# jaronlong52/neuron_poker

Measured on NVIDIA B200. Metric: showdown_evals_per_s, higher is better.
Workload: dtype u32

## Files before the change

### neuron_poker_b200/csrc/npk_device.cuh

```cuda
#pragma once
#include <cuda_runtime.h>
#include <stdint.h>

namespace npk {

constexpr int kDevDescShift = 9;
constexpr int kRowBits = 10;
constexpr uint32_t kColMask = (1u << kRowBits) - 1u;

struct DeviceTables {
    const uint16_t* value;
    const uint16_t* rowoff;
    const uint16_t* flush;
    const uint32_t* desc;
    uint32_t value_bytes;
    uint32_t rowoff_bytes;
    uint32_t flush_bytes;
    uint16_t type_start[10];
    uint32_t* check;
};

struct SmemTables {
    const uint16_t* value;
    const uint16_t* rowoff;
    const uint16_t* flush;
    const uint32_t* desc;
    uint32_t value_bytes, rowoff_bytes, flush_bytes;
    uint32_t* check;
};

#ifdef NPK_CHECKED
#define NPK_CHECK(ptr, cond, code) do { if (!(cond)) atomicMax((ptr), (unsigned)(code)); } while (0)
#else
#define NPK_CHECK(ptr, cond, code) do { } while (0)
#endif

constexpr uint32_t kDescBytes = 256;

__host__ __device__ __forceinline__ int validate_query(const uint8_t* hole, const uint8_t* board, int players,
                                                       unsigned long long* mask = nullptr)
{
    unsigned long long m = 0;
    int known = 0;
    bool bad = players < 1 || players > 10, ended = false;
    for (int i = 0; hole && i < 2; i++) {
        const int c = hole[i];
        if (c >= 52) bad = true; else { bad |= (m >> c & 1ull) != 0; m |= 1ull << c; }
    }
    for (int i = 0; i < 5; i++) {
        const int c = board[i];
        if (c == 0xFF) { ended = true; continue; }
        if (ended || c >= 52) { bad = true; continue; }
        bad |= (m >> c & 1ull) != 0;
        m |= 1ull << c;
        known++;
    }
    if (mask) *mask = m;
    return bad ? -1 : known;
}

__device__ __forceinline__ uint32_t smem_u32(const void* p) { return (uint32_t)__cvta_generic_to_shared(p); }

__device__ __forceinline__ void mbar_init(uint64_t* bar, uint32_t count)
{
    asm volatile("mbarrier.init.shared::cta.b64 [%0], %1;" ::"r"(smem_u32(bar)), "r"(count));
    asm volatile("fence.mbarrier_init.release.cluster;" ::: "memory");
}
__device__ __forceinline__ void mbar_expect_tx(uint64_t* bar, uint32_t bytes)
{
    asm volatile("mbarrier.arrive.expect_tx.shared::cta.b64 _, [%0], %1;" ::"r"(smem_u32(bar)), "r"(bytes) : "memory");
}
__device__ __forceinline__ void bulk_g2s(void* dst, const void* src, uint32_t bytes, uint64_t* bar)
{
    asm volatile("cp.async.bulk.shared::cluster.global.mbarrier::complete_tx::bytes [%0], [%1], %2, [%3];" ::"r"(
                     smem_u32(dst)),
                 "l"(src), "r"(bytes), "r"(smem_u32(bar))
                 : "memory");
}
__device__ __forceinline__ void mbar_wait(uint64_t* bar, uint32_t parity)
{
    uint32_t done = 0;
    while (!done) {
        asm volatile(
            "{\n .reg .pred p;\n mbarrier.try_wait.parity.shared::cta.b64 p, [%1], %2;\n selp.u32 %0, 1, 0, p;\n}\n"
            : "=r"(done)
            : "r"(smem_u32(bar)), "r"(parity)
            : "memory");
    }
}

__device__ __forceinline__ SmemTables stage_tables(const DeviceTables& t, uint8_t* base, uint64_t* bar)
{
    uint8_t* s_value = base;
    uint8_t* s_rowoff = s_value + t.value_bytes;
    uint8_t* s_flush = s_rowoff + t.rowoff_bytes;
    if (threadIdx.x == 0) mbar_init(bar, 1);
    __syncthreads();
    if (threadIdx.x == 0) {
        mbar_expect_tx(bar, t.value_bytes + t.rowoff_bytes + t.flush_bytes + kDescBytes);
        const uint32_t kChunk = 32768;
        for (uint32_t o = 0; o < t.value_bytes; o += kChunk)
            bulk_g2s(s_value + o, (const uint8_t*)t.value + o, min(kChunk, t.value_bytes - o), bar);
        bulk_g2s(s_rowoff, t.rowoff, t.rowoff_bytes, bar);
        bulk_g2s(s_flush, t.flush, t.flush_bytes, bar);
        bulk_g2s(s_flush + t.flush_bytes, t.desc, kDescBytes, bar);
    }
    mbar_wait(bar, 0);
    SmemTables s;
    s.value = (const uint16_t*)s_value;
    s.rowoff = (const uint16_t*)s_rowoff;
    s.flush = (const uint16_t*)s_flush;
    s.desc = (const uint32_t*)(s_flush + t.flush_bytes);
    s.value_bytes = t.value_bytes; s.rowoff_bytes = t.rowoff_bytes; s.flush_bytes = t.flush_bytes; s.check = t.check;
    return s;
}

__device__ __forceinline__ void philox4x32_10(uint32_t c0, uint32_t c1, uint32_t c2, uint32_t c3, uint32_t k0,
                                              uint32_t k1, uint32_t out[4])
{
    const uint32_t M0 = 0xD2511F53u, M1 = 0xCD9E8D57u, W0 = 0x9E3779B9u, W1 = 0xBB67AE85u;
#pragma unroll
    for (int r = 0; r < 10; r++) {
        uint64_t p0 = (uint64_t)M0 * c0, p1 = (uint64_t)M1 * c2;
        uint32_t n0 = (uint32_t)(p1 >> 32) ^ c1 ^ k0;
        uint32_t n2 = (uint32_t)(p0 >> 32) ^ c3 ^ k1;
        c1 = (uint32_t)p1;
        c3 = (uint32_t)p0;
        c0 = n0;
        c2 = n2;
        k0 += W0;
        k1 += W1;
    }
    out[0] = c0; out[1] = c1; out[2] = c2; out[3] = c3;
}

__device__ __forceinline__ uint32_t prmt(uint32_t a, uint32_t b, uint32_t sel)
{
    uint32_t r;
    asm("prmt.b32 %0, %1, %2, %3;" : "=r"(r) : "r"(a), "r"(b), "r"(sel));
    return r;
}

__device__ __forceinline__ uint32_t shr_clamp(uint32_t v, uint32_t n)
{
    uint32_t r;
    asm("shr.u32 %0, %1, %2;" : "=r"(r) : "r"(v), "r"(n));
    return r;
}

__device__ __forceinline__ uint32_t lds_u16(uint32_t saddr)
{
    uint32_t v;
    asm("ld.shared.u16 %0, [%1];" : "=r"(v) : "r"(saddr));
    return v;
}

struct SmemAddr {
    uint32_t value, rowoff, flush;
#ifdef NPK_CHECKED
    uint32_t value_bytes, rowoff_bytes, flush_bytes;
    uint32_t* check;
#endif
};

__device__ __forceinline__ SmemAddr smem_addr(const SmemTables& s)
{
    SmemAddr a;
    a.value = smem_u32(s.value); a.rowoff = smem_u32(s.rowoff); a.flush = smem_u32(s.flush);
#ifdef NPK_CHECKED
    a.value_bytes = s.value_bytes; a.rowoff_bytes = s.rowoff_bytes; a.flush_bytes = s.flush_bytes; a.check = s.check;
#endif
    return a;
}

__device__ __forceinline__ uint32_t lookup_nonflush(const SmemAddr& a, uint32_t total)
{
    const uint32_t row2 = __umulhi(total, 1u << (32 - (kDevDescShift + kRowBits - 1))) & (0xFFFFu << 1);
    NPK_CHECK(a.check, row2 + 2u <= a.rowoff_bytes, 1);
    const uint32_t off = lds_u16(a.rowoff + row2);
    const uint32_t col2 = __umulhi(total, 1u << (32 - (kDevDescShift - 1))) & (kColMask << 1);
    NPK_CHECK(a.check, col2 + (off << 1) + 2u <= a.value_bytes, 2);
    return lds_u16(a.value + col2 + (off << 1));
}

__device__ __forceinline__ uint32_t flush_bit(uint32_t d, uint32_t fsx) { return shr_clamp(0x1000u, (d ^ fsx) & 63u); }

__device__ __forceinline__ void card_bits(uint32_t d, uint32_t& lo, uint32_t& hi)
{
    const uint64_t b = 1ull << ((d & 0x30u) + 12u - (d & 15u));
    lo = (uint32_t)b;
    hi = (uint32_t)(b >> 32);
}

__device__ __forceinline__ uint32_t suit_inc(uint32_t d) { return 1u << ((d >> 2) & 12u); }

__device__ __forceinline__ uint32_t field_selector(uint32_t fs) { return 0x9910u + fs * 0x2222u; }

__device__ __forceinline__ uint32_t eval7_desc(const SmemAddr& a, const uint32_t d[7])
{
    uint32_t total = 0, cnt = 0x3333u;
#pragma unroll
    for (int i = 0; i < 7; i++) {
        total += d[i];
        cnt += suit_inc(d[i]);
    }
    uint32_t v = lookup_nonflush(a, total);
    const uint32_t f = cnt & 0x8888u;
    if (f) {
        const uint32_t fsx = (((31u - __clz(f)) >> 2) & 3u) << 4;
        uint32_t field = 0;
#pragma unroll
        for (int i = 0; i < 7; i++) field |= shr_clamp(0x1000u, (d[i] ^ fsx) & 63u);
        NPK_CHECK(a.check, 2u * field + 2u <= a.flush_bytes, 3);
        v = lds_u16(a.flush + 2u * field);
    }
    return v;
}

}
```

### neuron_poker_b200/csrc/npk_kernels.cu

```cuda
#include <atomic>
#include <cstdlib>
#include "npk_mc.cuh"

namespace npk {

template <int NOPP, int NB, int REF>
__device__ __forceinline__ void shape_kernel_body(const EquityParams& p)
{
    extern __shared__ __align__(128) uint8_t smem[];
    const WarpCtx cx = warp_context(p, smem, 64 + (45 + NB) * 32);
    const int lane = cx.lane;
    const long long n_items = p.nq * p.chunks;
    for (long long item = next_item(p.work_counter, lane); item < n_items; item = next_item(p.work_counter, lane)) {
        long long q, t_begin, t_end;
        item_range(p, item, q, t_begin, t_end);
        if (REF) refdeal_item<NOPP, NB>(p, cx, q, t_begin, t_end);
        else uniform_item<NOPP, NB>(p, cx, q, t_begin, t_end);
    }
    finish_single_call(p, lane);
    if (p.peer) finish_peer(p.peer, p.peer_epoch, p.peer_totals, p.peer_words, lane);
}

template <int NOPP, int NB>
__global__ void __launch_bounds__(kEquityMaxThreads, 1) equity_uniform_kernel(const EquityParams p)
{
    shape_kernel_body<NOPP, NB, 0>(p);
}

template <int NOPP, int NB>
__global__ void __launch_bounds__(kEquityMaxThreads, 1) equity_refdeal_kernel(const EquityParams p)
{
    shape_kernel_body<NOPP, NB, 1>(p);
}

__device__ __forceinline__ bool class_allowed(const uint32_t (&mask)[6], int c1, int c2)
{
    const int r1 = c1 >> 2, r2 = c2 >> 2, hi = max(r1, r2), lo = min(r1, r2);
    const int k = ((c1 ^ c2) & 3) == 0 ? hi * 13 + lo : lo * 13 + hi;
    return (mask[k >> 5] >> (k & 31)) & 1u;
}

template <int MODE>
__global__ void __launch_bounds__(kRefThreads, 1) equity_ranges_kernel(const EquityParams p)
{
    extern __shared__ __align__(128) uint8_t smem[];
    uint64_t* bar = reinterpret_cast<uint64_t*>(smem);
    const SmemAddr st = smem_addr(stage_tables(p.tables, smem + 128, bar));
    const int lane = threadIdx.x & 31;

    const long long n_items = p.nq * p.chunks;

    for (long long item = next_item(p.work_counter, lane); item < n_items; item = next_item(p.work_counter, lane)) {
        long long q, t_begin, t_end;
        item_range(p, item, q, t_begin, t_end);
        int known = 0;
        for (int i = 0; i < 5; i++) known += p.board[5 * q + i] != 0xFF;
        const int nknown = (int)p.n_known;
        const int nopp = max(0, (int)p.n_players[q] - 1 - nknown);

        uint64_t taken = 0;
        uint32_t board_sum = 0, board_lo = 0, board_hi = 0, board_cnt = 0x5555u;
        for (int i = 0; i < known; i++) {
            const uint8_t c = p.board[5 * q + i];
            const uint32_t d = p.tables.desc[c];
            uint32_t l, h;
            card_bits(d, l, h);
            board_sum += d; board_lo |= l; board_hi |= h; board_cnt += suit_inc(d);
            taken |= 1ull << c;
        }
        if (p.ghost)
            for (int i = 0; i < 2; i++) { const uint8_t c = p.ghost[2 * q + i]; if (c < 52) taken |= 1ull << c; }
        int h0 = 0, h1 = 0;
        if (!p.hero_range) { h0 = p.hole[2 * q]; h1 = p.hole[2 * q + 1]; taken |= (1ull << h0) | (1ull << h1); }
        for (int f = 0; f < 2 * nknown; f++) taken |= 1ull << (p.known_opp[2 * q * nknown + f] & 63u);
        const uint64_t avail0 = ~taken & ((1ull << 52) - 1ull);
        const int n0 = __popcll(avail0);

        uint32_t wins = 0, ties = 0;
        unsigned long long passes = 0;
        unsigned long long wt_pack = 0;

        for (long long tb = t_begin; tb < t_end; tb += 32) {
            if (*reinterpret_cast<volatile uint32_t*>(p.abort_flag)) break;
            const long long t_local = tb + lane;
            bool active = t_local < t_end;
            const unsigned long long trial = (unsigned long long)(p.trial_offset + t_local);
            WordStream rs;
            rs.c0 = (uint32_t)trial; rs.c1 = (uint32_t)(trial >> 32); rs.c2 = (uint32_t)q + p.query_offset;
            rs.k0 = p.seed_lo; rs.k1 = p.seed_hi; rs.blk = MODE == 1 ? 0x80000000u : 0xC0000000u; rs.have = 0;

            uint64_t avail = avail0;
            int n = n0;
            uint32_t hd0 = 0, hd1 = 0, best = 0;
            uint32_t oc1[9], oc2[9];
            if (active) {
                for (int o = p.hero_range ? -1 : 0; o < nopp && active; o++) {
                    const bool is_hero = o < 0;
                    int c1 = 0, c2 = 0;
                    uint32_t tries = 0;
                    for (;;) {
                        if (++tries > kMaxRangeAttempts) { atomicExch(p.abort_flag, 1u); active = false; break; }
                        passes++;
                        const uint64_t prod = (uint64_t)rs.next() * (uint32_t)n;
                        const uint32_t i1 = (uint32_t)(prod >> 32);
                        const uint32_t i2 = __umulhi((uint32_t)prod, (uint32_t)(n - 1));
                        if (MODE == 1 && i1 == i2) continue;
                        c1 = select_bit(avail, (int)i1);
                        if (MODE == 1) {
                            const int ct = select_bit(avail, (int)i2);
                            if (!(is_hero ? class_allowed(p.hero_mask, c1, ct) : class_allowed(p.opp_mask, c1, ct))) continue;
                            c2 = is_hero ? ct : select_bit(avail & ~(1ull << c1), (int)i2);
                        } else {
                            c2 = select_bit(avail & ~(1ull << c1), (int)i2);
                            if (!(is_hero ? class_allowed(p.hero_mask, c1, c2) : class_allowed(p.opp_mask, c1, c2))) continue;
                        }
                        break;
                    }
                    avail &= ~((1ull << c1) | (1ull << c2));
                    n -= 2;
                    if (is_hero) { h0 = c1; h1 = c2; }
                    else { oc1[o] = p.tables.desc[c1]; oc2[o] = p.tables.desc[c2]; }
                }
            }
            hd0 = p.tables.desc[h0]; hd1 = p.tables.desc[h1];
            uint32_t bsum = board_sum, bcnt = board_cnt;
            uint32_t bd[5];
            int nbd = 0;
            if (active) {
                for (int k = known; k < 5; k++) {
                    const uint32_t j = __umulhi(rs.next(), (uint32_t)(MODE == 1 ? n - 1 : n));
                    const int c = select_bit(avail, (int)j);
                    avail &= ~(1ull << c);
                    n--;
                    const uint32_t d = p.tables.desc[c];
                    bd[nbd++] = d;
                    bsum += d; bcnt += suit_inc(d);
                }
            }
            const BoardFlush bf = board_flush(bcnt);
            uint32_t bfield = prmt(board_lo, board_hi, bf.sel);
            for (int k = 0; k < nbd; k++) bfield |= flush_bit(bd[k], bf.fsx);
            const uint32_t hv = eval_player(st, bsum + hd0 + hd1, bfield | flush_bit(hd0, bf.fsx) | flush_bit(hd1, bf.fsx), bf.thr);
            if (active) {
                for (int o = 0; o < nopp; o++)
                    best = max(best, eval_player(st, bsum + oc1[o] + oc2[o],
                                                 bfield | flush_bit(oc1[o], bf.fsx) | flush_bit(oc2[o], bf.fsx), bf.thr));
                for (int f = 0; f < nknown; f++) {
                    const uint32_t k1 = p.tables.desc[p.known_opp[2 * (q * nknown + f)] & 63u];
                    const uint32_t k2 = p.tables.desc[p.known_opp[2 * (q * nknown + f) + 1] & 63u];
                    best = max(best, eval_player(st, bsum + k1 + k2, bfield | flush_bit(k1, bf.fsx) | flush_bit(k2, bf.fsx), bf.thr));
                }
            }
            const int nrivals = nopp + nknown;
            const bool win = active && (nrivals == 0 || hv > best), tie = active && nrivals > 0 && hv == best;
            wins += win; ties += tie;
            if (p.win_types && (win || tie)) {
                uint32_t ty = 0;
#pragma unroll
                for (int i = 1; i < 9; i++) ty += hv >= p.tables.type_start[i];
                wt_pack += 1ull << (7 * ty);
            }
        }
        wins = __reduce_add_sync(0xffffffffu, wins);
        ties = __reduce_add_sync(0xffffffffu, ties);
        if (lane == 0) {
            atomicAdd(&p.wins[q], (unsigned long long)wins);
            atomicAdd(&p.ties[q], (unsigned long long)ties);
        }
        if (p.passes) {
            unsigned long long tot = 0;
#pragma unroll
            for (int sft = 0; sft < 63; sft += 21)
                tot += (unsigned long long)__reduce_add_sync(0xffffffffu, (uint32_t)(passes >> sft) & 0x1fffffu) << sft;
            if (lane == 0) atomicAdd(&p.passes[q], tot);
        }
        if (p.win_types) {
#pragma unroll
            for (int i = 0; i < 9; i++) {
                uint32_t c = __reduce_add_sync(0xffffffffu, (uint32_t)(wt_pack >> (7 * i)) & 127u);
                if (lane == 0 && c) atomicAdd(&p.win_types[9 * q + i], (unsigned long long)c);
            }
        }
    }
}

__global__ void __launch_bounds__(kRank7Threads, 1) rank7_kernel(const DeviceTables tables, const uint8_t* __restrict__ cards,
                                                               long long n, uint16_t* __restrict__ out)
{
    extern __shared__ __align__(128) uint8_t smem[];
    uint64_t* bar = reinterpret_cast<uint64_t*>(smem);
    const SmemAddr st = smem_addr(stage_tables(tables, smem + 128, bar));
    uint8_t* extra = smem + 128 + tables.value_bytes + tables.rowoff_bytes + tables.flush_bytes + kDescBytes;
    uint2* s_card = reinterpret_cast<uint2*>(extra);
    for (int i = threadIdx.x; i < 64 * 32; i += blockDim.x) {
        const int c = i >> 5;
        const uint32_t d = c < 52 ? tables.desc[c] : 0u;
        s_card[i] = make_uint2(d, c < 52 ? suit_inc(d) : 0u);
    }
    __syncthreads();
    const uint32_t lane_base = smem_u32(s_card) + 8u * (threadIdx.x & 31);
    auto card_entry = [&](uint32_t w, int k) {
        const uint32_t f = w & (0x3Fu << (8 * k));
        uint32_t addr;
        if (k == 0) addr = f * 256u + lane_base;
        else if (k == 1) addr = f + lane_base;
        else asm("mad.hi.u32 %0, %1, %2, %3;" : "=r"(addr) : "r"(f), "r"(1u << (32 - (8 * k - 8))), "r"(lane_base));
        uint2 e;
        asm("ld.shared.v2.u32 {%0, %1}, [%2];" : "=r"(e.x), "=r"(e.y) : "r"(addr));
        return e;
    };
    auto eval7 = [&](const uint2 (&e)[7]) {
        const uint32_t total = (e[0].x + e[1].x + e[2].x) + (e[3].x + e[4].x + e[5].x) + e[6].x;
        const uint32_t cnt = (0x3333u + e[0].y + e[1].y) + (e[2].y + e[3].y + e[4].y) + (e[5].y + e[6].y);
        uint32_t v = lookup_nonflush(st, total);
        const uint32_t f = cnt & 0x8888u;
        if (f) {
            const uint32_t fsx = (((31u - __clz(f)) >> 2) & 3u) << 4;
            uint32_t field = 0;
#pragma unroll
            for (int i = 0; i < 7; i++) field |= shr_clamp(0x1000u, (e[i].x ^ fsx) & 63u);
            NPK_CHECK(st.check, 2u * field + 2u <= st.flush_bytes, 3);
            v = lds_u16(st.flush + 2u * field);
        }
        return v;
    };
    const bool aligned = ((reinterpret_cast<uintptr_t>(cards) & 3u) == 0) && ((reinterpret_cast<uintptr_t>(out) & 7u) == 0);
    const long long quads = aligned ? n / 4 : 0;
    const uint32_t* __restrict__ words = reinterpret_cast<const uint32_t*>(cards);
    const long long stride = (long long)gridDim.x * blockDim.x;
    long long g = (long long)blockIdx.x * blockDim.x + threadIdx.x;
    uint32_t nxt[7];
    if (g < quads) {
#pragma unroll
        for (int k = 0; k < 7; k++) nxt[k] = __ldg(words + 7 * g + k);
    }
    for (; g < quads; g += stride) {
        uint32_t w[7];
#pragma unroll
        for (int k = 0; k < 7; k++) w[k] = nxt[k];
        if (g + stride < quads) {
#pragma unroll
            for (int k = 0; k < 7; k++) nxt[k] = __ldg(words + 7 * (g + stride) + k);
        }
        uint32_t r[4];
#pragma unroll
        for (int h = 0; h < 4; h++) {
            uint2 e[7];
#pragma unroll
            for (int k = 0; k < 7; k++) {
                const int byte = 7 * h + k;
                e[k] = card_entry(w[byte >> 2], byte & 3);
            }
            r[h] = eval7(e);
        }
        uint2 packed;
        packed.x = r[0] | (r[1] << 16);
        packed.y = r[2] | (r[3] << 16);
        *reinterpret_cast<uint2*>(out + 4 * g) = packed;
    }
    for (long long i = 4 * quads + (long long)blockIdx.x * blockDim.x + threadIdx.x; i < n; i += (long long)gridDim.x * blockDim.x) {
        uint2 e[7];
#pragma unroll
        for (int k = 0; k < 7; k++) e[k] = card_entry(cards[7 * i + k], 0);
        out[i] = (uint16_t)eval7(e);
    }
}

__device__ __forceinline__ unsigned long long binom(int n, int k)
{
    if (k < 0 || k > n) return 0;
    unsigned long long r = 1;
    for (int i = 1; i <= k; i++) r = r * (unsigned long long)(n - k + i) / (unsigned long long)i;
    return r;
}

__global__ void __launch_bounds__(kAuxThreads, 1) rank7_colex_kernel(const DeviceTables tables, long long first,
                                                                     long long count, uint16_t* __restrict__ out)
{
    extern __shared__ __align__(128) uint8_t smem[];
    uint64_t* bar = reinterpret_cast<uint64_t*>(smem);
    const SmemAddr st = smem_addr(stage_tables(tables, smem + 128, bar));
    uint32_t* s_desc = reinterpret_cast<uint32_t*>(smem + 128 + tables.value_bytes + tables.rowoff_bytes + tables.flush_bytes);
    if (threadIdx.x < 52) s_desc[threadIdx.x] = tables.desc[threadIdx.x];
    __syncthreads();
    for (long long i = (long long)blockIdx.x * blockDim.x + threadIdx.x; i < count; i += (long long)gridDim.x * blockDim.x) {
        unsigned long long r = (unsigned long long)(first + i);
        uint32_t d[7];
        int hi = 51;
#pragma unroll
        for (int k = 7; k >= 1; k--) {
            int c = hi;
            while (binom(c, k) > r) c--;
            r -= binom(c, k);
            d[k - 1] = s_desc[c];
            hi = c - 1;
        }
        out[i] = (uint16_t)eval7_desc(st, d);
    }
}

__global__ void __launch_bounds__(kAuxThreads, 1) enum_kernel(const EnumParams p)
{
    extern __shared__ __align__(128) uint8_t smem[];
    uint64_t* bar = reinterpret_cast<uint64_t*>(smem);
    const SmemAddr st = smem_addr(stage_tables(p.tables, smem + 128, bar));
    uint8_t* extra = smem + 128 + p.tables.value_bytes + p.tables.rowoff_bytes + p.tables.flush_bytes;
    uint32_t* s_deck = reinterpret_cast<uint32_t*>(extra);
    uint16_t* s_pairval = reinterpret_cast<uint16_t*>(extra + 256);
    uint16_t* s_pair = reinterpret_cast<uint16_t*>(extra + 256 + 2688);
    __shared__ unsigned long long s_acc[3];
    const int warp = threadIdx.x >> 5, lane = threadIdx.x & 31, nwarps = blockDim.x >> 5;

    for (int i = threadIdx.x; i < 1326; i += blockDim.x) {
        int b = (int)((1.0f + sqrtf(1.0f + 8.0f * (float)i)) * 0.5f);
        while (b * (b - 1) / 2 > i) b--;
        while ((b + 1) * b / 2 <= i) b++;
        s_pair[i] = (uint16_t)((i - b * (b - 1) / 2) | b << 8);
    }

    for (long long q = blockIdx.x; q < p.nq; q += gridDim.x) {
// ... 321 lines not shown
```

### neuron_poker_b200/csrc/npk_mc.cuh

```cuda
#pragma once
#include "npk_device.cuh"
#include "npk_kernels.h"

namespace npk {

__device__ __forceinline__ long long next_item(unsigned long long* counter, int lane)
{
    unsigned long long it = 0;
    if (lane == 0) it = atomicAdd(counter, 1ull);
    return (long long)__shfl_sync(0xffffffffu, it, 0);
}

__device__ __forceinline__ void item_range(const EquityParams& p, long long item, long long& qslot, long long& begin, long long& end)
{
    qslot = item / p.chunks;
    begin = (item - qslot * p.chunks) * p.chunk;
    end = min(p.trials, begin + (long long)p.chunk);
}

struct QueryStatic {
    uint32_t hero_sum;
    uint32_t hero_lo, hero_hi;
    uint32_t board_sum;
    uint32_t board_lo, board_hi;
    uint32_t board_cnt;
    uint64_t known;
};

__device__ __forceinline__ QueryStatic load_query(const EquityParams& p, const uint32_t* sdesc, long long q, int nb_known)
{
    QueryStatic s;
    const uint8_t h0 = p.hole ? p.hole[2 * q] : (uint8_t)p.inline_query;
    const uint8_t h1 = p.hole ? p.hole[2 * q + 1] : (uint8_t)(p.inline_query >> 8);
    uint32_t d0 = sdesc[h0], d1 = sdesc[h1], l, h;
    s.hero_sum = d0 + d1;
    card_bits(d0, s.hero_lo, s.hero_hi);
    card_bits(d1, l, h);
    s.hero_lo |= l; s.hero_hi |= h;
    s.known = (1ull << h0) | (1ull << h1);
    s.board_sum = 0; s.board_lo = 0; s.board_hi = 0; s.board_cnt = 0x5555u;
    for (int i = 0; i < nb_known; i++) {
        const uint8_t c = p.hole ? p.board[5 * q + i] : (uint8_t)(p.inline_query >> (16 + 8 * i));
        uint32_t d = sdesc[c];
        card_bits(d, l, h);
        s.board_sum += d; s.board_lo |= l; s.board_hi |= h; s.board_cnt += suit_inc(d);
        s.known |= 1ull << c;
    }
    return s;
}

__device__ __forceinline__ void finish_single_call(const EquityParams& p, int lane)
{
    SingleCall* sc = p.single;
    if (!sc) return;
    __syncwarp();
    unsigned int last = 0;
    if (lane == 0) {
        __threadfence();
        const unsigned int total = gridDim.x * (blockDim.x >> 5);
        last = atomicAdd(&sc->ticket, 1u) == total - 1u;
    }
    last = __shfl_sync(0xffffffffu, last, 0);
    if (!last) return;
    __threadfence();
    unsigned long long v = 0;
    if (lane < 12) {
        unsigned long long* src = &sc->wins;
        v = atomicExch(src + lane, 0ull);
    }
    if (lane == 0) { sc->work_counter = 0; sc->ticket = 0; }
    if (lane < 12) (&sc->host->wins)[lane] = v;
    __threadfence_system();
    __syncwarp();
    if (lane == 0) *reinterpret_cast<volatile unsigned long long*>(&sc->host->seq) = p.single_seq;
}

static __device__ __noinline__ void finish_peer(PeerCall* pc, unsigned long long epoch, unsigned long long* totals, uint32_t words,
                                         int lane)
{
    __syncwarp();
    unsigned int last = 0;
    if (lane == 0) {
        __threadfence();
        const unsigned int total = gridDim.x * (blockDim.x >> 5);
        last = atomicAdd(&pc->ticket, 1u) == total - 1u;
    }
    last = __shfl_sync(0xffffffffu, last, 0);
    if (!last) return;
    __threadfence();
    const uint32_t world = pc->world, me = pc->rank;
    const uint32_t parity = (uint32_t)(epoch & 1ull);
    const size_t my_slot = ((size_t)parity * world + me) * pc->stride;
    for (uint32_t base = 0; base < words; base += 128) {
        unsigned long long v[4];
#pragma unroll
        for (int k = 0; k < 4; k++) {
            const uint32_t i = base + 32u * k + lane;
            v[k] = i < words ? atomicExch(&pc->acc[i], 0ull) : 0ull;
        }
        for (uint32_t r = 0; r < world; r++) {
            unsigned long long* dst = pc->slots[r] + my_slot;
#pragma unroll
            for (int k = 0; k < 4; k++) {
                const uint32_t i = base + 32u * k + lane;
                if (i < words) dst[i] = v[k];
            }
        }
    }
    __threadfence_system();
    __syncwarp();
    if (lane < world)
        asm volatile("st.release.sys.global.u64 [%0], %1;" ::"l"(pc->flags[lane] + parity * kMaxPeers + me), "l"(epoch) : "memory");
    if (lane < world) {
        const unsigned long long* f = pc->flags[me] + parity * kMaxPeers + lane;
        const long long t0 = clock64();
        unsigned long long seen;
        for (;;) {
            asm volatile("ld.acquire.sys.global.u64 %0, [%1];" : "=l"(seen) : "l"(f) : "memory");
            if (seen >= epoch) break;
            if (clock64() - t0 > (4ll << 30)) { pc->error = 1u; break; }
        }
    }
    __syncwarp();
    const unsigned long long* mine = pc->slots[me] + (size_t)parity * world * pc->stride;
    for (uint32_t base = 0; base < words; base += 128) {
        unsigned long long sum[4] = {0, 0, 0, 0};
#pragma unroll 4
        for (uint32_t r = 0; r < world; r++) {
#pragma unroll
            for (int k = 0; k < 4; k++) {
                const uint32_t i = base + 32u * k + lane;
                if (i < words) sum[k] += __ldcg(mine + (size_t)r * pc->stride + i);
            }
        }
#pragma unroll
        for (int k = 0; k < 4; k++) {
            const uint32_t i = base + 32u * k + lane;
            if (i < words) totals[i] = sum[k];
        }
    }
    if (lane == 0) { pc->work_counter = 0; pc->ticket = 0; }
}

struct BoardFlush {
    uint32_t fsx;
    uint32_t sel;
    uint32_t thr;
};

__device__ __forceinline__ BoardFlush board_flush(uint32_t board_cnt)
{
    BoardFlush b;
    const uint32_t f = board_cnt & 0x8888u;
    const uint32_t fs = ((31u - __clz(f)) >> 2) & 3u;
    b.fsx = fs << 4;
    b.sel = field_selector(fs);
    b.thr = f ? 5u : 64u;
    return b;
}

__device__ __forceinline__ uint32_t eval_player(const SmemAddr& a, uint32_t total, uint32_t field, uint32_t thr)
{
    uint32_t v = lookup_nonflush(a, total);
    NPK_CHECK(a.check, 2u * field + 2u <= a.flush_bytes, 3);
    if ((uint32_t)__popc(field) >= thr) v = max(v, lds_u16(a.flush + 2u * field));
    return v;
}

__device__ __forceinline__ uint32_t lds_u32(uint32_t saddr)
{
    uint32_t v;
    asm volatile("ld.shared.u32 %0, [%1];" : "=r"(v) : "r"(saddr) : "memory");
    return v;
}
__device__ __forceinline__ void sts_u32(uint32_t saddr, uint32_t v)
{
    asm volatile("st.shared.u32 [%0], %1;" ::"r"(saddr), "r"(v) : "memory");
}

struct WarpCtx {
    SmemAddr st;
    const uint32_t* sdesc;
    uint32_t* scratch;
    uint32_t fy_addr;
    int lane;
};

__device__ __forceinline__ WarpCtx warp_context(const EquityParams& p, uint8_t* smem, int words_per_warp)
{
    uint64_t* bar = reinterpret_cast<uint64_t*>(smem);
    const SmemTables stab = stage_tables(p.tables, smem + 128, bar);
    const uint32_t table_bytes = 128 + p.tables.value_bytes + p.tables.rowoff_bytes + p.tables.flush_bytes + kDescBytes;
    const int warp = threadIdx.x >> 5, lane = threadIdx.x & 31;
    WarpCtx cx;
    cx.st = smem_addr(stab);
    cx.sdesc = stab.desc;
    cx.scratch = reinterpret_cast<uint32_t*>(smem + table_bytes) + warp * words_per_warp;
    cx.fy_addr = smem_u32(cx.scratch + 64 + lane);
    cx.lane = lane;
    return cx;
}

template <int NOPP, int NB>
__device__ __forceinline__ void uniform_item(const EquityParams& p, const WarpCtx& cx, long long q, long long t_begin,
            long long t_end)
{
    constexpr int KNOWN = 5 - NB;
    constexpr int N = 50 - KNOWN;
    constexpr int D = 2 * NOPP + NB;
    constexpr int NW = (D + 1) / 2;
    constexpr int NBLK2 = (2 * NW + 3) / 4;
    static_assert(D <= N, "not enough cards");

    const SmemAddr& st = cx.st;
    const int lane = cx.lane;
    uint32_t* scratch = cx.scratch;
    uint32_t* fy = scratch + 64 + lane;
    const uint32_t fy_addr = cx.fy_addr;
    const QueryStatic qs = load_query(p, cx.sdesc, q, KNOWN);

    __syncwarp();
    {
        const uint64_t avail = ~qs.known & ((1ull << 52) - 1ull);
        for (int c = lane; c < 52; c += 32)
            if (avail >> c & 1ull) scratch[__popcll(avail & ((1ull << c) - 1ull))] = cx.sdesc[c];
    }
    __syncwarp();
#pragma unroll 4
    for (int j = 0; j < N; j++) fy[j * 32] = scratch[j];
    __syncwarp();

    const unsigned long long a_begin = (unsigned long long)(p.trial_offset + t_begin);
    const unsigned long long a_end = (unsigned long long)(p.trial_offset + t_end);
    uint32_t wins = 0, ties = 0;
    unsigned long long wt_pack = 0;

    const uint32_t span = (uint32_t)(a_end - a_begin);
    uint32_t rel = (uint32_t)(2ull * (a_begin >> 1) - a_begin) + 2u * (uint32_t)lane;
    for (unsigned long long pb = a_begin >> 1; pb <= (a_end - 1) >> 1; pb += 32, rel += 64u) {
        const unsigned long long pair = pb + lane;
        uint32_t w[NBLK2 > 0 ? NBLK2 * 4 : 1];
#pragma unroll
        for (int b = 0; b < NBLK2; b++)
            philox4x32_10((uint32_t)pair, (uint32_t)(pair >> 32), (uint32_t)q + p.query_offset, (uint32_t)b,
                          p.seed_lo, p.seed_hi, &w[4 * b]);
        uint32_t dv[2][D > 0 ? D : 1];
#pragma unroll
        for (int u = 0; u < 2; u++) {
            uint32_t slot[D > 0 ? D : 1];
            uint32_t rem = 0;
#pragma unroll
            for (int k = 0; k < D; k++) {
                const uint32_t x = (k & 1) ? rem : w[u * NW + (k >> 1)];
                const uint32_t idx = __umulhi(x, (uint32_t)(N - k));
                rem = x * (uint32_t)(N - k);
                slot[k] = fy_addr + idx * 128u;
                dv[u][k] = lds_u32(slot[k]);
                sts_u32(slot[k], lds_u32(fy_addr + (uint32_t)(N - 1 - k) * 128u));
            }
#pragma unroll
            for (int k = D - 1; k >= 0; k--) sts_u32(slot[k], dv[u][k]);
        }
#pragma unroll
        for (int u = 0; u < 2; u++) {
            const bool active = rel + (uint32_t)u < span;
            uint32_t bsum = qs.board_sum, bcnt = qs.board_cnt;
#pragma unroll
            for (int k = 2 * NOPP; k < D; k++) { bsum += dv[u][k]; bcnt += suit_inc(dv[u][k]); }
            const BoardFlush bf = board_flush(bcnt);
            uint32_t bfield = prmt(qs.board_lo, qs.board_hi, bf.sel);
#pragma unroll
            for (int k = 2 * NOPP; k < D; k++) bfield |= flush_bit(dv[u][k], bf.fsx);
            const uint32_t hv = eval_player(st, bsum + qs.hero_sum, bfield | prmt(qs.hero_lo, qs.hero_hi, bf.sel), bf.thr);
            uint32_t best = 0;
#pragma unroll
            for (int o = 0; o < NOPP; o++) {
                const uint32_t d0 = dv[u][2 * o], d1 = dv[u][2 * o + 1];
                best = max(best, eval_player(st, bsum + d0 + d1, bfield | flush_bit(d0, bf.fsx) | flush_bit(d1, bf.fsx), bf.thr));
            }
            const bool win = active && (NOPP == 0 || hv > best), tie = active && NOPP > 0 && hv == best;
            wins += win; ties += tie;
            if (p.win_types && (win || tie)) {
                uint32_t ty = 0;
#pragma unroll
                for (int i = 1; i < 9; i++) ty += hv >= p.tables.type_start[i];
                wt_pack += 1ull << (7 * ty);
            }
        }
    }
#ifdef NPK_CHECKED
    __syncwarp();
    for (int j = 0; j < N; j++) NPK_CHECK(st.check, fy[j * 32] == scratch[j], 7);
#endif
    wins = __reduce_add_sync(0xffffffffu, wins);
    ties = __reduce_add_sync(0xffffffffu, ties);
    if (lane == 0) {
        atomicAdd(&p.wins[q], (unsigned long long)wins);
        atomicAdd(&p.ties[q], (unsigned long long)ties);
    }
    if (p.win_types) {
#pragma unroll
        for (int i = 0; i < 9; i++) {
            uint32_t c = __reduce_add_sync(0xffffffffu, (uint32_t)(wt_pack >> (7 * i)) & 127u);
            if (lane == 0 && c) atomicAdd(&p.win_types[9 * q + i], (unsigned long long)c);
        }
    }
}


struct WordStream {
    uint32_t c0, c1, c2, k0, k1, blk, have;
    uint32_t w[4];
    __device__ __forceinline__ uint32_t next()
    {
        if (have == 0) { philox4x32_10(c0, c1, c2, blk++, k0, k1, w); have = 4; }
        const uint32_t r = w[0];
        w[0] = w[1]; w[1] = w[2]; w[2] = w[3];
        have--;
        return r;
    }
};

__device__ __forceinline__ int select_bit(uint64_t m, int k)
{
    uint32_t lo = (uint32_t)m, hi = (uint32_t)(m >> 32);
    int c = __popc(lo), base = 0;
    uint32_t w = lo;
    if (k >= c) { k -= c; w = hi; base = 32; }
#pragma unroll
    for (int s = 16; s >= 1; s >>= 1) {
        const uint32_t lowmask = (1u << s) - 1u;
        const int cl = __popc(w & lowmask);
        if (k >= cl) { k -= cl; w >>= s; base += s; } else { w &= lowmask; }
    }
    return base;
}

__device__ __forceinline__ uint32_t bump4(uint32_t x4, uint32_t c, uint32_t h)
{
    const uint32_t t = (x4 + c) & h;
    return x4 + (t >> 7);
}

template <int D>
__device__ __forceinline__ void lehmer_decode(const uint32_t (&raw)[D > 0 ? D : 1], uint32_t (&x4)[(D + 3) / 4 > 0 ? (D + 3) / 4 : 1])
{
    constexpr int G = (D + 3) / 4;
#pragma unroll
    for (int g = 0; g < G; g++) {
        uint32_t v = raw[4 * g];
#pragma unroll
        for (int b = 1; b < 4; b++)
            if (4 * g + b < D) v += raw[4 * g + b] << (8 * b);
        x4[g] = v;
    }
#pragma unroll
    for (int k = D - 2; k >= 0; k--) {
        const uint32_t c = 0x80808080u - raw[k] * 0x01010101u;
#pragma unroll
        for (int g = (k + 1) / 4; g < G; g++) {
            uint32_t h = 0;
#pragma unroll
            for (int b = 0; b < 4; b++)
                if (4 * g + b > k && 4 * g + b < D) h |= 0x80u << (8 * b);
            x4[g] = bump4(x4[g], c, h);
        }
    }
}

__device__ __forceinline__ uint32_t slot_addr(uint32_t x4, int b, uint32_t base)
{
    const uint32_t f = x4 & (0xFFu << (8 * b));
    return b == 0 ? base + f * 128u : base + (f >> (8 * b - 7));
}

template <int NOPP, int NB>
__device__ __forceinline__ void refdeal_item(const EquityParams& p, const WarpCtx& cx, long long q, long long t_begin,
            long long t_end)
{
    constexpr int KNOWN = 5 - NB;
    constexpr int N = 50 - KNOWN;
    constexpr int D = 2 * NOPP + NB;
    constexpr int NWR = NOPP + (NB + 1) / 2;
    constexpr int NBLK2 = (2 * NWR + 3) / 4;
    constexpr int G = (D + 3) / 4;
    static_assert(D <= N, "not enough cards");

    const SmemAddr& st = cx.st;
    const int lane = cx.lane;
    uint32_t* scratch = cx.scratch;
    uint32_t* fy = scratch + 64 + lane;
    const uint32_t fy_addr = cx.fy_addr;
    const QueryStatic qs = load_query(p, cx.sdesc, q, KNOWN);

    __syncwarp();
    {
        const uint64_t avail = ~qs.known & ((1ull << 52) - 1ull);
        for (int c = lane; c < 52; c += 32)
            if (avail >> c & 1ull) scratch[__popcll(avail & ((1ull << c) - 1ull))] = cx.sdesc[c];
    }
    __syncwarp();
#pragma unroll 4
    for (int j = 0; j < N; j++) fy[j * 32] = scratch[j];
    __syncwarp();

    const unsigned long long a_begin = (unsigned long long)(p.trial_offset + t_begin);
    const unsigned long long a_end = (unsigned long long)(p.trial_offset + t_end);
    uint32_t wins = 0, ties = 0, passes = 0;
    unsigned long long wt_pack = 0;

    const uint32_t span = (uint32_t)(a_end - a_begin);
    uint32_t rel = (uint32_t)(2ull * (a_begin >> 1) - a_begin) + 2u * (uint32_t)lane;
    for (unsigned long long pb = a_begin >> 1; pb <= (a_end - 1) >> 1; pb += 32, rel += 64u) {
        const unsigned long long pair = pb + lane;
        uint32_t w[NBLK2 > 0 ? NBLK2 * 4 : 1];
#pragma unroll
        for (int b = 0; b < NBLK2; b++)
            philox4x32_10((uint32_t)pair, (uint32_t)(pair >> 32), (uint32_t)q + p.query_offset, 0x80000000u + (uint32_t)b,
                          p.seed_lo, p.seed_hi, &w[4 * b]);
        uint32_t dv[2][D > 0 ? D : 1];
#pragma unroll
        for (int u = 0; u < 2; u++) {
            uint32_t raw[D > 0 ? D : 1];
#pragma unroll
            for (int o = 0; o < NOPP; o++) {
                const uint32_t m = (uint32_t)(N - 2 * o - 1);
                const uint32_t x = w[u * NWR + o];
                const uint32_t a = __umulhi(x, m), b = __umulhi(x * m, m);
                raw[2 * o] = a + (a >= b ? 1u : 0u);
                raw[2 * o + 1] = b;
            }
            uint32_t rem = 0;
#pragma unroll
            for (int c = 0; c < NB; c++) {
                const uint32_t m = (uint32_t)(N - 2 * NOPP - c - 1);
                const uint32_t x = (c & 1) ? rem : w[u * NWR + NOPP + (c >> 1)];
                raw[2 * NOPP + c] = __umulhi(x, m);
                rem = x * m;
            }
            uint32_t x4[G > 0 ? G : 1];
            lehmer_decode<D>(raw, x4);
#pragma unroll
            for (int k = 0; k < D; k++) dv[u][k] = lds_u32(slot_addr(x4[k >> 2], k & 3, fy_addr));
        }
        if (p.passes) {
            constexpr int NPB = (2 * NOPP + 3) / 4;
#pragma unroll
            for (int b = 0; b < NPB; b++) {
                uint32_t pw[4];
                philox4x32_10((uint32_t)pair, (uint32_t)(pair >> 32), (uint32_t)q + p.query_offset, 0x40000000u + (uint32_t)b,
                              p.seed_lo, p.seed_hi, pw);
#pragma unroll
                for (int i = 0; i < 4; i++) {
                    const int s = 4 * b + i;
                    if (s < 2 * NOPP) {
                        const uint32_t n = (uint32_t)(N - 2 * (s % (NOPP > 0 ? NOPP : 1)));
                        uint32_t x = pw[i], tries = 1;
                        while (x < 0xFFFFFFFFu / n && tries < kMaxRangeAttempts) { tries++; x *= n; }
                        if (rel + (uint32_t)(s / (NOPP > 0 ? NOPP : 1)) < span) passes += tries;
                    }
                }
            }
        }
#pragma unroll
        for (int u = 0; u < 2; u++) {
            const bool active = rel + (uint32_t)u < span;
            uint32_t bsum = qs.board_sum, bcnt = qs.board_cnt;
#pragma unroll
            for (int k = 2 * NOPP; k < D; k++) { bsum += dv[u][k]; bcnt += suit_inc(dv[u][k]); }
            const BoardFlush bf = board_flush(bcnt);
            uint32_t bfield = prmt(qs.board_lo, qs.board_hi, bf.sel);
#pragma unroll
            for (int k = 2 * NOPP; k < D; k++) bfield |= flush_bit(dv[u][k], bf.fsx);
            const uint32_t hv = eval_player(st, bsum + qs.hero_sum, bfield | prmt(qs.hero_lo, qs.hero_hi, bf.sel), bf.thr);
            uint32_t best = 0;
#pragma unroll
            for (int o = 0; o < NOPP; o++) {
                const uint32_t d0 = dv[u][2 * o], d1 = dv[u][2 * o + 1];
                best = max(best, eval_player(st, bsum + d0 + d1, bfield | flush_bit(d0, bf.fsx) | flush_bit(d1, bf.fsx), bf.thr));
            }
            const bool win = active && (NOPP == 0 || hv > best), tie = active && NOPP > 0 && hv == best;
            wins += win; ties += tie;
            if (p.win_types && (win || tie)) {
                uint32_t ty = 0;
#pragma unroll
                for (int i = 1; i < 9; i++) ty += hv >= p.tables.type_start[i];
                wt_pack += 1ull << (7 * ty);
            }
        }
    }

    wins = __reduce_add_sync(0xffffffffu, wins);
    ties = __reduce_add_sync(0xffffffffu, ties);
    if (lane == 0) {
        atomicAdd(&p.wins[q], (unsigned long long)wins);
        atomicAdd(&p.ties[q], (unsigned long long)ties);
    }
    if (p.passes) {
        const uint32_t plo = __reduce_add_sync(0xffffffffu, passes & 0xffffu);
        const uint32_t phi = __reduce_add_sync(0xffffffffu, passes >> 16);
        if (lane == 0) atomicAdd(&p.passes[q], (unsigned long long)plo + ((unsigned long long)phi << 16));
    }
    if (p.win_types) {
#pragma unroll
        for (int i = 0; i < 9; i++) {
            uint32_t c = __reduce_add_sync(0xffffffffu, (uint32_t)(wt_pack >> (7 * i)) & 127u);
            if (lane == 0 && c) atomicAdd(&p.win_types[9 * q + i], (unsigned long long)c);
        }
    }
}


}
```

### neuron_poker_b200/csrc/npk_mixed.cu

```cuda
#include "npk_mc.cuh"

namespace npk {

template <int NOPP, int NB, int REF>
__device__ __noinline__ void shape_item(const EquityParams* p, const WarpCtx* cx, long long q, long long t_begin, long long t_end)
{
    const EquityParams lp = *p;
    const WarpCtx lcx = *cx;
    if (REF) refdeal_item<NOPP, NB>(lp, lcx, q, t_begin, t_end);
    else uniform_item<NOPP, NB>(lp, lcx, q, t_begin, t_end);
}

template <int NOPP, int REF>
__device__ __forceinline__ void dispatch_known(int known, const EquityParams* p, const WarpCtx* cx, long long q, long long b,
                                               long long e)
{
    switch (known) {
        case 0: shape_item<NOPP, 5, REF>(p, cx, q, b, e); break;
        case 1: shape_item<NOPP, 4, REF>(p, cx, q, b, e); break;
        case 2: shape_item<NOPP, 3, REF>(p, cx, q, b, e); break;
        case 3: shape_item<NOPP, 2, REF>(p, cx, q, b, e); break;
        case 4: shape_item<NOPP, 1, REF>(p, cx, q, b, e); break;
        default: shape_item<NOPP, 0, REF>(p, cx, q, b, e); break;
    }
}

template <int REF>
__global__ void __launch_bounds__(kMixedThreads, 1) equity_mixed_kernel(const EquityParams p)
{
    extern __shared__ __align__(128) uint8_t smem[];
    __shared__ long long s_first[kShapeGroups + 1];
    const WarpCtx cx = warp_context(p, smem, 64 + 50 * 32);
    const int lane = cx.lane;
    const uint32_t* counts = p.group;
    const long long per_query = p.chunks;
    if (threadIdx.x == 0) {
        long long acc = 0;
        for (int g = 0; g < kShapeGroups; g++) { s_first[g] = acc; acc += (long long)counts[g] * per_query; }
        s_first[kShapeGroups] = acc;
    }
    __syncthreads();
    const long long n_items = s_first[kShapeGroups];
    for (long long item = next_item(p.work_counter, lane); item < n_items; item = next_item(p.work_counter, lane)) {
        uint32_t before = 0;
        if (lane < kShapeGroups) before += item >= s_first[lane + 1];
        if (lane + 32 < kShapeGroups) before += item >= s_first[lane + 33];
        const int g = (int)__reduce_add_sync(0xffffffffu, before);
        long long qslot, t_begin, t_end;
        item_range(p, item - s_first[g], qslot, t_begin, t_end);
        const long long q = p.qindex[counts[64 + g] + qslot];
        const int known = g % 6;
        switch (g / 6) {
            case 0: dispatch_known<0, REF>(known, &p, &cx, q, t_begin, t_end); break;
            case 1: dispatch_known<1, REF>(known, &p, &cx, q, t_begin, t_end); break;
            case 2: dispatch_known<2, REF>(known, &p, &cx, q, t_begin, t_end); break;
            case 3: dispatch_known<3, REF>(known, &p, &cx, q, t_begin, t_end); break;
            case 4: dispatch_known<4, REF>(known, &p, &cx, q, t_begin, t_end); break;
            case 5: dispatch_known<5, REF>(known, &p, &cx, q, t_begin, t_end); break;
            case 6: dispatch_known<6, REF>(known, &p, &cx, q, t_begin, t_end); break;
            case 7: dispatch_known<7, REF>(known, &p, &cx, q, t_begin, t_end); break;
            case 8: dispatch_known<8, REF>(known, &p, &cx, q, t_begin, t_end); break;
            default: dispatch_known<9, REF>(known, &p, &cx, q, t_begin, t_end); break;
        }
    }
}

__device__ __forceinline__ uint4 ld_volatile_v4(const void* p)
{
    uint4 v;
    asm volatile("ld.volatile.global.v4.u32 {%0, %1, %2, %3}, [%4];" : "=r"(v.x), "=r"(v.y), "=r"(v.z), "=r"(v.w) : "l"(p) : "memory");
    return v;
}
__device__ __forceinline__ void st_volatile_v4(void* p, uint4 v)
{
    asm volatile("st.volatile.global.v4.u32 [%0], {%1, %2, %3, %4};" ::"l"(p), "r"(v.x), "r"(v.y), "r"(v.z), "r"(v.w) : "memory");
}

template <int REF>
__device__ __forceinline__ void dispatch_players(int players, int known, const EquityParams* p, const WarpCtx* cx, long long b,
                                                 long long e)
{
    switch (players - 1) {
        case 0: dispatch_known<0, REF>(known, p, cx, 0, b, e); break;
        case 1: dispatch_known<1, REF>(known, p, cx, 0, b, e); break;
        case 2: dispatch_known<2, REF>(known, p, cx, 0, b, e); break;
        case 3: dispatch_known<3, REF>(known, p, cx, 0, b, e); break;
        case 4: dispatch_known<4, REF>(known, p, cx, 0, b, e); break;
        case 5: dispatch_known<5, REF>(known, p, cx, 0, b, e); break;
        case 6: dispatch_known<6, REF>(known, p, cx, 0, b, e); break;
        case 7: dispatch_known<7, REF>(known, p, cx, 0, b, e); break;
        case 8: dispatch_known<8, REF>(known, p, cx, 0, b, e); break;
        default: dispatch_known<9, REF>(known, p, cx, 0, b, e); break;
    }
}

__device__ __forceinline__ void serve_request(EquityParams& p, const WarpCtx& cx, const uint4 a, const uint4 b,
                                              unsigned long long* s_cnt, unsigned long long* acc, ResidentMailbox* mb)
{
    const int warp = threadIdx.x >> 5, warps = blockDim.x >> 5;
    const unsigned int total_warps = gridDim.x * warps;
    const unsigned int trials = a.y, hi = a.w;
    unsigned int chunk = trials / (8u * total_warps);
    chunk = (chunk + 63u) / 64u * 64u;
    chunk = chunk < 64u ? 64u : (chunk > 2048u ? 2048u : chunk);
    const unsigned int chunks = (trials + chunk - 1u) / chunk;
    const int players = (int)(hi >> 24 & 15u);
    const unsigned long long packed = (unsigned long long)a.z | (unsigned long long)(hi & 0xFFFFFFu) << 32;
    int known = 0;
#pragma unroll
    for (int i = 0; i < 5; i++) known += (packed >> (16 + 8 * i) & 0xFFull) != 0xFFull;
    p.hole = nullptr; p.inline_query = packed;
    p.trials = trials; p.trial_offset = 0; p.query_offset = 0;
    p.seed_lo = b.y; p.seed_hi = b.z;
    p.chunk = chunk; p.chunks = chunks;
    p.wins = &s_cnt[0]; p.ties = &s_cnt[1];
    for (unsigned int item = warp * gridDim.x + blockIdx.x; item < chunks; item += total_warps) {
        const long long t_begin = (long long)item * chunk;
        const long long t_end = min((long long)trials, t_begin + (long long)chunk);
        if (hi >> 31) dispatch_players<1>(players, known, &p, &cx, t_begin, t_end);
        else dispatch_players<0>(players, known, &p, &cx, t_begin, t_end);
    }
    __syncthreads();
    if (threadIdx.x == 0) {
        const unsigned long long mine = s_cnt[0] | s_cnt[1] << 28 | 1ull << 56;
        const unsigned long long old = atomicAdd(acc, mine);
        if ((old >> 56) == gridDim.x - 1u) {
            const unsigned long long tot = old + mine;
            asm volatile("st.global.v4.u32 [%0], {%1, %2, %3, %4};" ::"l"(&mb->done), "r"((unsigned int)(tot & 0xFFFFFFFu)),
                         "r"((unsigned int)(tot >> 28 & 0xFFFFFFFu)), "r"(b.w), "r"(0u)
                         : "memory");
        }
    }
}

__global__ void __launch_bounds__(kMixedThreads, 1)
equity_resident_kernel(const DeviceTables tables, ResidentState* st, ResidentMailbox* mb, const unsigned long long launch_id,
                       const unsigned int last_seq, const long long idle_cycles)
{
    extern __shared__ __align__(128) uint8_t smem[];
    __shared__ uint4 s_a, s_b;
    __shared__ unsigned long long s_cnt[2];
    EquityParams p{};
    p.tables = tables;
    const WarpCtx cx = warp_context(p, smem, 64 + 50 * 32);
    unsigned int cmd = 0;
    unsigned int seq_seen = last_seq;
    long long t_last = clock64();
    for (;;) {
        if (threadIdx.x == 0) {
            uint4 a, b;
            if (blockIdx.x == 0) {
                bool leave = false;
                for (;;) {
                    a = ld_volatile_v4(&mb->a);
                    b = ld_volatile_v4(&mb->b);
                    if (a.x == b.x && a.x != seq_seen) break;
                    if (b.w == (unsigned int)launch_id || clock64() - t_last > idle_cycles) { leave = true; break; }
                }
                seq_seen = leave ? seq_seen : a.x;
                a.x = cmd + 1; b.w = leave ? 0u : b.x; b.x = cmd + 1;
                st_volatile_v4(&st->a, a);
                st_volatile_v4(&st->b, b);
            } else {
                do {
                    a = ld_volatile_v4(&st->a);
                    b = ld_volatile_v4(&st->b);
                } while (a.x != cmd + 1 || b.x != cmd + 1);
            }
            s_a = a; s_b = b;
            s_cnt[0] = 0; s_cnt[1] = 0;
        }
        __syncthreads();
        cmd++;
        const uint4 a = s_a, b = s_b;
        if (b.w == 0u) break;
        serve_request(p, cx, a, b, s_cnt, &st->acc[cmd & 1], mb);
        if (threadIdx.x == 0) {
            if (blockIdx.x == 0) {
                st->acc[(cmd + 1) & 1] = 0;
                __threadfence();
            }
            t_last = clock64();
        }
    }
    if (blockIdx.x == 0 && threadIdx.x == 0) {
        __threadfence_system();
        *reinterpret_cast<volatile unsigned long long*>(&mb->exited) = launch_id;
    }
}

__global__ void __launch_bounds__(kMixedThreads, 1)
equity_oneshot_kernel(const DeviceTables tables, ResidentState* st, ResidentMailbox* mb, const uint4 a, const uint4 b,
                      const unsigned int parity)
{
    extern __shared__ __align__(128) uint8_t smem[];
    __shared__ unsigned long long s_cnt[2];
    EquityParams p{};
    p.tables = tables;
    if (threadIdx.x == 0) {
        s_cnt[0] = 0; s_cnt[1] = 0;
        if (blockIdx.x == 0) st->acc[parity ^ 1u] = 0;
    }
    const WarpCtx cx = warp_context(p, smem, 64 + 50 * 32);
    serve_request(p, cx, a, b, s_cnt, &st->acc[parity], mb);
}

cudaError_t launch_equity_resident(const DeviceTables& t, ResidentState* st, ResidentMailbox* mb, unsigned long long launch_id,
                                   unsigned int last_seq, long long idle_cycles, int ctas, cudaStream_t s)
{
    const size_t fixed = 128 + (size_t)t.value_bytes + t.rowoff_bytes + t.flush_bytes + kDescBytes;
    const size_t smem = fixed + (size_t)(kMixedThreads / 32) * (64 + 50 * 32) * 4;
    cudaError_t e = cudaFuncSetAttribute(equity_resident_kernel, cudaFuncAttributeMaxDynamicSharedMemorySize, (int)smem);
    if (e != cudaSuccess) return e;
    equity_resident_kernel<<<ctas, kMixedThreads, smem, s>>>(t, st, mb, launch_id, last_seq, idle_cycles);
    return cudaGetLastError();
}

cudaError_t launch_equity_oneshot(const DeviceTables& t, ResidentState* st, ResidentMailbox* mb, uint4 a, uint4 b,
                                  unsigned int parity, int sm_count, cudaStream_t s)
{
    const long long items = ((long long)a.y + 63) / 64;
    const int warps = items <= 4ll * sm_count ? 4 : kMixedThreads / 32;
    long long grid = (items + warps - 1) / warps;
    if (grid < 1) grid = 1;
    if (grid > sm_count) grid = sm_count;
    if (grid > 255) grid = 255;
    const size_t fixed = 128 + (size_t)t.value_bytes + t.rowoff_bytes + t.flush_bytes + kDescBytes;
    const size_t smem_max = fixed + (size_t)(kMixedThreads / 32) * (64 + 50 * 32) * 4;
    const size_t smem = fixed + (size_t)warps * (64 + 50 * 32) * 4;
    static bool opted[64];
    int dev = 0;
    cudaGetDevice(&dev);
    if (dev < 0 || dev >= 64 || !opted[dev]) {
        cudaError_t e = cudaFuncSetAttribute(equity_oneshot_kernel, cudaFuncAttributeMaxDynamicSharedMemorySize, (int)smem_max);
        if (e != cudaSuccess) return e;
        if (dev >= 0 && dev < 64) opted[dev] = true;
    }
    equity_oneshot_kernel<<<(int)grid, warps * 32, smem, s>>>(t, st, mb, a, b, parity);
    return cudaGetLastError();
}

cudaError_t launch_equity_mixed(const EquityParams& p, int sm_count, cudaStream_t s)
{
    auto k = p.reference_dealer ? equity_mixed_kernel<1> : equity_mixed_kernel<0>;
    const size_t fixed = 128 + (size_t)p.tables.value_bytes + p.tables.rowoff_bytes + p.tables.flush_bytes + kDescBytes;
    const size_t smem = fixed + (size_t)(kMixedThreads / 32) * (64 + 50 * 32) * 4;
    cudaError_t e = cudaFuncSetAttribute(k, cudaFuncAttributeMaxDynamicSharedMemorySize, (int)smem);
    if (e != cudaSuccess) return e;
    k<<<sm_count, kMixedThreads, smem, s>>>(p);
    return cudaGetLastError();
}

}
```

Measured before the change: 460.9 billion.

## Skip remaining opponent lookups once hero is already beaten in showdown

Factors the per-deal showdown into a helper and, on the uniform path of the main kernel, evaluates only the first one or two opponents unconditionally. The remaining opponents' table loads are predicated on the hero still being at least as strong as the best so far, so shared-memory lookups are skipped once the hero has lost. It also drops the redundant Fisher-Yates swap and restore for the last dealt card. This trades fewer shared-memory loads for predicated inline asm and some warp divergence; results stay exact because a lost hand stays lost.

```diff
diff --git a/neuron_poker_b200/csrc/npk_device.cuh b/neuron_poker_b200/csrc/npk_device.cuh
--- a/neuron_poker_b200/csrc/npk_device.cuh
+++ b/neuron_poker_b200/csrc/npk_device.cuh
@@ -155,6 +155,18 @@
     return v;
 }
 
+__device__ __forceinline__ uint32_t lds_u16_if(uint32_t v, uint32_t saddr, bool live)
+{
+    asm("{\n .reg .pred p;\n setp.ne.u32 p, %2, 0;\n @p ld.shared.u16 %0, [%1];\n}" : "+r"(v) : "r"(saddr), "r"((uint32_t)live));
+    return v;
+}
+__device__ __forceinline__ uint32_t lds_u16_max_if(uint32_t best, uint32_t saddr, bool live)
+{
+    asm("{\n .reg .pred p;\n .reg .u32 t;\n setp.ne.u32 p, %2, 0;\n @p ld.shared.u16 t, [%1];\n @p max.u32 %0, %0, t;\n}"
+        : "+r"(best) : "r"(saddr), "r"((uint32_t)live));
+    return best;
+}
+
 struct SmemAddr {
     uint32_t value, rowoff, flush;
 #ifdef NPK_CHECKED
@@ -181,6 +193,16 @@
     const uint32_t col2 = __umulhi(total, 1u << (32 - (kDevDescShift - 1))) & (kColMask << 1);
     NPK_CHECK(a.check, col2 + (off << 1) + 2u <= a.value_bytes, 2);
     return lds_u16(a.value + col2 + (off << 1));
+}
+
+__device__ __forceinline__ uint32_t lookup_nonflush_max_if(const SmemAddr& a, uint32_t total, uint32_t best, bool live)
+{
+    const uint32_t row2 = __umulhi(total, 1u << (32 - (kDevDescShift + kRowBits - 1))) & (0xFFFFu << 1);
+    NPK_CHECK(a.check, !live || row2 + 2u <= a.rowoff_bytes, 1);
+    const uint32_t off = lds_u16_if(row2, a.rowoff + row2, live);
+    const uint32_t col2 = __umulhi(total, 1u << (32 - (kDevDescShift - 1))) & (kColMask << 1);
+    NPK_CHECK(a.check, !live || col2 + (off << 1) + 2u <= a.value_bytes, 2);
+    return lds_u16_max_if(best, a.value + col2 + (off << 1), live);
 }
 
 __device__ __forceinline__ uint32_t flush_bit(uint32_t d, uint32_t fsx) { return shr_clamp(0x1000u, (d ^ fsx) & 63u); }
diff --git a/neuron_poker_b200/csrc/npk_kernels.cu b/neuron_poker_b200/csrc/npk_kernels.cu
--- a/neuron_poker_b200/csrc/npk_kernels.cu
+++ b/neuron_poker_b200/csrc/npk_kernels.cu
@@ -14,8 +14,8 @@
     for (long long item = next_item(p.work_counter, lane); item < n_items; item = next_item(p.work_counter, lane)) {
         long long q, t_begin, t_end;
         item_range(p, item, q, t_begin, t_end);
-        if (REF) refdeal_item<NOPP, NB>(p, cx, q, t_begin, t_end);
-        else uniform_item<NOPP, NB>(p, cx, q, t_begin, t_end);
+        if (REF) refdeal_item<NOPP, NB, false>(p, cx, q, t_begin, t_end);
+        else uniform_item<NOPP, NB, true>(p, cx, q, t_begin, t_end);
     }
     finish_single_call(p, lane);
     if (p.peer) finish_peer(p.peer, p.peer_epoch, p.peer_totals, p.peer_words, lane);
diff --git a/neuron_poker_b200/csrc/npk_mc.cuh b/neuron_poker_b200/csrc/npk_mc.cuh
--- a/neuron_poker_b200/csrc/npk_mc.cuh
+++ b/neuron_poker_b200/csrc/npk_mc.cuh
@@ -167,6 +167,54 @@
     return v;
 }
 
+__device__ __forceinline__ uint32_t eval_player_max_if(const SmemAddr& a, uint32_t total, uint32_t field, uint32_t thr,
+                                                       uint32_t best, bool live)
+{
+    best = lookup_nonflush_max_if(a, total, best, live);
+    NPK_CHECK(a.check, 2u * field + 2u <= a.flush_bytes, 3);
+    return lds_u16_max_if(best, a.flush + 2u * field, live && (uint32_t)__popc(field) >= thr);
+}
+
+template <int NOPP>
+constexpr int kUngatedOpponents = NOPP < 8 ? (NOPP < 1 ? NOPP : 1) : 2;
+
+template <int NOPP, int NB, bool GATED>
+__device__ __forceinline__ void showdown(const EquityParams& p, const SmemAddr& st, const QueryStatic& qs,
+                                         const uint32_t (&dv)[2 * NOPP + NB > 0 ? 2 * NOPP + NB : 1], bool active,
+                                         uint32_t& wins, uint32_t& ties, unsigned long long& wt_pack)
+{
+    constexpr int D = 2 * NOPP + NB;
+    constexpr int NA = GATED ? kUngatedOpponents<NOPP> : NOPP;
+    uint32_t bsum = qs.board_sum, bcnt = qs.board_cnt;
+#pragma unroll
+    for (int k = 2 * NOPP; k < D; k++) { bsum += dv[k]; bcnt += suit_inc(dv[k]); }
+    const BoardFlush bf = board_flush(bcnt);
+    uint32_t bfield = prmt(qs.board_lo, qs.board_hi, bf.sel);
+#pragma unroll
+    for (int k = 2 * NOPP; k < D; k++) bfield |= flush_bit(dv[k], bf.fsx);
+    const uint32_t hv = eval_player(st, bsum + qs.hero_sum, bfield | prmt(qs.hero_lo, qs.hero_hi, bf.sel), bf.thr);
+    uint32_t best = 0;
+#pragma unroll
+    for (int o = 0; o < NA; o++) {
+        const uint32_t d0 = dv[2 * o], d1 = dv[2 * o + 1];
+        best = max(best, eval_player(st, bsum + d0 + d1, bfield | flush_bit(d0, bf.fsx) | flush_bit(d1, bf.fsx), bf.thr));
+    }
+    const bool live = hv >= best;
+#pragma unroll
+    for (int o = NA; o < NOPP; o++) {
+        const uint32_t d0 = dv[2 * o], d1 = dv[2 * o + 1];
+        best = eval_player_max_if(st, bsum + d0 + d1, bfield | flush_bit(d0, bf.fsx) | flush_bit(d1, bf.fsx), bf.thr, best, live);
+    }
+    const bool win = active && (NOPP == 0 || hv > best), tie = active && NOPP > 0 && hv == best;
+    wins += win; ties += tie;
+    if (p.win_types && (win || tie)) {
+        uint32_t ty = 0;
+#pragma unroll
+        for (int i = 1; i < 9; i++) ty += hv >= p.tables.type_start[i];
+        wt_pack += 1ull << (7 * ty);
+    }
+}
+
 __device__ __forceinline__ uint32_t lds_u32(uint32_t saddr)
 {
     uint32_t v;
@@ -201,7 +249,7 @@
     return cx;
 }
 
-template <int NOPP, int NB>
+template <int NOPP, int NB, bool GATED>
 __device__ __forceinline__ void uniform_item(const EquityParams& p, const WarpCtx& cx, long long q, long long t_begin,
             long long t_end)
 {
@@ -256,37 +304,13 @@
                 rem = x * (uint32_t)(N - k);
                 slot[k] = fy_addr + idx * 128u;
                 dv[u][k] = lds_u32(slot[k]);
-                sts_u32(slot[k], lds_u32(fy_addr + (uint32_t)(N - 1 - k) * 128u));
+                if (k < D - 1) sts_u32(slot[k], lds_u32(fy_addr + (uint32_t)(N - 1 - k) * 128u));
             }
 #pragma unroll
-            for (int k = D - 1; k >= 0; k--) sts_u32(slot[k], dv[u][k]);
-        }
-#pragma unroll
-        for (int u = 0; u < 2; u++) {
-            const bool active = rel + (uint32_t)u < span;
-            uint32_t bsum = qs.board_sum, bcnt = qs.board_cnt;
-#pragma unroll
-            for (int k = 2 * NOPP; k < D; k++) { bsum += dv[u][k]; bcnt += suit_inc(dv[u][k]); }
-            const BoardFlush bf = board_flush(bcnt);
-            uint32_t bfield = prmt(qs.board_lo, qs.board_hi, bf.sel);
-#pragma unroll
-            for (int k = 2 * NOPP; k < D; k++) bfield |= flush_bit(dv[u][k], bf.fsx);
-            const uint32_t hv = eval_player(st, bsum + qs.hero_sum, bfield | prmt(qs.hero_lo, qs.hero_hi, bf.sel), bf.thr);
-            uint32_t best = 0;
-#pragma unroll
-            for (int o = 0; o < NOPP; o++) {
-                const uint32_t d0 = dv[u][2 * o], d1 = dv[u][2 * o + 1];
-                best = max(best, eval_player(st, bsum + d0 + d1, bfield | flush_bit(d0, bf.fsx) | flush_bit(d1, bf.fsx), bf.thr));
-            }
-            const bool win = active && (NOPP == 0 || hv > best), tie = active && NOPP > 0 && hv == best;
-            wins += win; ties += tie;
-            if (p.win_types && (win || tie)) {
-                uint32_t ty = 0;
-#pragma unroll
-                for (int i = 1; i < 9; i++) ty += hv >= p.tables.type_start[i];
-                wt_pack += 1ull << (7 * ty);
-            }
-        }
+            for (int k = D - 2; k >= 0; k--) sts_u32(slot[k], dv[u][k]);
+        }
+#pragma unroll
+        for (int u = 0; u < 2; u++) showdown<NOPP, NB, GATED>(p, st, qs, dv[u], rel + (uint32_t)u < span, wins, ties, wt_pack);
     }
 #ifdef NPK_CHECKED
     __syncwarp();
@@ -374,7 +398,7 @@
     return b == 0 ? base + f * 128u : base + (f >> (8 * b - 7));
 }
 
-template <int NOPP, int NB>
+template <int NOPP, int NB, bool GATED>
 __device__ __forceinline__ void refdeal_item(const EquityParams& p, const WarpCtx& cx, long long q, long long t_begin,
             long long t_end)
 {
@@ -463,31 +487,7 @@
             }
         }
 #pragma unroll
-        for (int u = 0; u < 2; u++) {
-            const bool active = rel + (uint32_t)u < span;
-            uint32_t bsum = qs.board_sum, bcnt = qs.board_cnt;
-#pragma unroll
-            for (int k = 2 * NOPP; k < D; k++) { bsum += dv[u][k]; bcnt += suit_inc(dv[u][k]); }
-            const BoardFlush bf = board_flush(bcnt);
-            uint32_t bfield = prmt(qs.board_lo, qs.board_hi, bf.sel);
-#pragma unroll
-            for (int k = 2 * NOPP; k < D; k++) bfield |= flush_bit(dv[u][k], bf.fsx);
-            const uint32_t hv = eval_player(st, bsum + qs.hero_sum, bfield | prmt(qs.hero_lo, qs.hero_hi, bf.sel), bf.thr);
-            uint32_t best = 0;
-#pragma unroll
-            for (int o = 0; o < NOPP; o++) {
-                const uint32_t d0 = dv[u][2 * o], d1 = dv[u][2 * o + 1];
-                best = max(best, eval_player(st, bsum + d0 + d1, bfield | flush_bit(d0, bf.fsx) | flush_bit(d1, bf.fsx), bf.thr));
-            }
-            const bool win = active && (NOPP == 0 || hv > best), tie = active && NOPP > 0 && hv == best;
-            wins += win; ties += tie;
-            if (p.win_types && (win || tie)) {
-                uint32_t ty = 0;
-#pragma unroll
-                for (int i = 1; i < 9; i++) ty += hv >= p.tables.type_start[i];
-                wt_pack += 1ull << (7 * ty);
-            }
-        }
+        for (int u = 0; u < 2; u++) showdown<NOPP, NB, GATED>(p, st, qs, dv[u], rel + (uint32_t)u < span, wins, ties, wt_pack);
     }
 
     wins = __reduce_add_sync(0xffffffffu, wins);
diff --git a/neuron_poker_b200/csrc/npk_mixed.cu b/neuron_poker_b200/csrc/npk_mixed.cu
--- a/neuron_poker_b200/csrc/npk_mixed.cu
+++ b/neuron_poker_b200/csrc/npk_mixed.cu
@@ -7,8 +7,8 @@
 {
     const EquityParams lp = *p;
     const WarpCtx lcx = *cx;
-    if (REF) refdeal_item<NOPP, NB>(lp, lcx, q, t_begin, t_end);
-    else uniform_item<NOPP, NB>(lp, lcx, q, t_begin, t_end);
+    if (REF) refdeal_item<NOPP, NB, false>(lp, lcx, q, t_begin, t_end);
+    else uniform_item<NOPP, NB, false>(lp, lcx, q, t_begin, t_end);
 }
 
 template <int NOPP, int REF>
```

Result: faster. 468.3 billion, median of 6 (+1.6%).
